# Agricultural-Robotics-Bonn/pagnerf

Hardware: AMD Instinct MI355X
Metric: rays/sec (train step) on BUP20-shape scene (higher is better)
Workload: dtype bf16

## Files before the change

### include/pagnerf_hip.h

```cpp
#ifndef PAGNERF_HIP_H
#define PAGNERF_HIP_H

#include <stdint.h>

#ifdef __cplusplus
extern "C" {
#endif

#define PAG_ABI_VERSION 14

enum { PAG_F32 = 0, PAG_F16 = 1, PAG_BF16 = 2 };
enum { PAG_OK = 0, PAG_ERR_ARG = -1, PAG_ERR_LAUNCH = -2, PAG_ERR_UNSUPPORTED = -3 };
enum { PAG_ACT_NONE = 0, PAG_ACT_SIGMOID = 1, PAG_ACT_SOFTMAX = 2 };
enum { PAG_MLP_MFMA_BF16 = 0, PAG_MLP_FP32 = 1 };
enum { PAG_BG_BLACK = 0, PAG_BG_WHITE = 1 };
enum { PAG_LAYOUT_STRIDED = 0, PAG_LAYOUT_XCD8 = 1 };
enum { PAG_ENC_HALF_COORDS = 1 };
#define PAG_MAX_LEVELS 32
#define PAG_MAX_FEATS 64

int pag_abi_version(void);
const char *pag_last_error_string(void);


// ... 91 lines not shown
    void *dz[3];
    void *dx1; int dx1_dtype;
    int mode;
    const float *g_ray; const float *g_scale; const int32_t *g_index;
    const float *softmax_stats; const float *b_last;
    int dx1_accumulate;
    const float *dx1_col0_add;
    const float *dx1_col0_gate;
    const float *g_ray_scale;
    const void *x1; int x1_dtype; const float *x2; int k2p; const int32_t *x2_index;
    float *wgrad_workspace; int64_t wgrad_workspace_bytes;
    float *dW[3]; float *db[3];
    const float *b[3];
    const struct pag_mlp_bwd_args *pair;
    float *dz0_slots;
} pag_mlp_bwd_args;
int pag_mlp_bwd(const pag_mlp_bwd_args *args, int64_t M, void *stream);
int64_t pag_mlp_dz0_slots_bytes(int64_t M, int64_t R);
int pag_mlp_dz0_slots_sum(const int64_t *pack_start, int64_t R, const float *slots, float *out, void *stream);
int pag_mlp_bwd_fused_supported(const pag_mlp_bwd_args *args);
#define PAG_MLP_FUSED_WIDE_MAX_M ((int64_t)1 << 24)
int64_t pag_mlp_bwd_fused_workspace_bytes(const pag_mlp_bwd_args *args, int64_t M);
int pag_mlp_bwd_pair_supported(const pag_mlp_bwd_args *args, const pag_mlp_bwd_args *pair);

int pag_affine_xcd8_fwd(const void *x, int64_t M, int x_levels, int x_feats, const float *W, const float *b, int n_out, int in_dim,
                        float *out, void *stream);
int pag_affine_xcd8_bwd_dx(const float *grad_out, int64_t M, int x_levels, int x_feats, const float *W, int n_out, int in_dim, void *dx,
                           void *stream);

int pag_head_composite_fwd(const int64_t *pack_start, const int32_t *ray_of_pack, int64_t P,
                           const void *hidden, const float *W_last, const float *b_last, int out_dim,
                           const float *softmax_stats, const float *weights, const float *alpha,
                           float *out, int64_t n_samples, void *stream);

int pag_mlp_wgrad_blocks(int64_t M);
int pag_mlp_wgrad(const void *dz, int dz_cols, int n_out, const void *a1, int a1_dtype,
                  int a1_layout, int k1, const float *a2, int k2p, const int32_t *a2_index, int n_in,
                  float *slabs, int n_blocks, int64_t M, void *stream);
// ... 290 lines not shown
```

### pagnerf_amd/_lib.py

```python
import ctypes
import os

import torch

from . import build as _build

F32, F16, BF16 = 0, 1, 2
I32, I64 = 3, 4
ACT_NONE, ACT_SIGMOID, ACT_SOFTMAX = 0, 1, 2
MLP_MFMA_BF16, MLP_FP32 = 0, 1
BG_BLACK, BG_WHITE = 0, 1
LAYOUT_STRIDED, LAYOUT_XCD8 = 0, 1
ENC_HALF_COORDS = 1
ABI_VERSION = 14
MLP_FUSED_WIDE_MAX_M = 1 << 24

_DT = {torch.float32: F32, torch.float16: F16, torch.bfloat16: BF16}

c_i64, c_i32, c_u32, c_f32, c_vp = ctypes.c_int64, ctypes.c_int, ctypes.c_uint32, ctypes.c_float, ctypes.c_void_p
c_fp = ctypes.POINTER(ctypes.c_float)
c_ip = ctypes.POINTER(ctypes.c_int)


class HeadCompositeArgs(ctypes.Structure):
# ... 31 lines not shown

MlpBwdArgs._fields_ = [("grad_out", c_vp), ("out", c_vp), ("out_dtype", c_i32), ("out_act", c_i32),
                ("k1", c_i32), ("in_dim", c_i32), ("n_layers", c_i32), ("out_dim", c_i32),
                ("x1_layout", c_i32), ("x1_levels", c_i32), ("x1_feats", c_i32),
                ("W", c_vp * 3),
                ("hidden_save", c_vp * 2),
                ("dz", c_vp * 3),
                ("dx1", c_vp), ("dx1_dtype", c_i32),
                ("mode", c_i32),
                ("g_ray", c_vp), ("g_scale", c_vp), ("g_index", c_vp),
                ("softmax_stats", c_vp), ("b_last", c_vp), ("dx1_accumulate", c_i32), ("dx1_col0_add", c_vp),
                ("dx1_col0_gate", c_vp), ("g_ray_scale", c_vp),
                ("x1", c_vp), ("x1_dtype", c_i32), ("x2", c_vp), ("k2p", c_i32), ("x2_index", c_vp),
                ("wgrad_workspace", c_vp), ("wgrad_workspace_bytes", c_i64),
                ("dW", c_vp * 3), ("db", c_vp * 3), ("b", c_vp * 3),
                ("pair", ctypes.POINTER(MlpBwdArgs)), ("dz0_slots", c_vp)]


class DeepMlpArgs(ctypes.Structure):
    _fields_ = [("coords", c_vp), ("ray_d", c_vp), ("hidden", c_i32), ("num_classes", c_i32), ("channels", c_i32), ("save", c_i32),
                ("W", c_vp * 14), ("b", c_vp * 14), ("density", c_vp), ("rgb", c_vp), ("semantics", c_vp),
                ("workspace", c_vp), ("workspace_bytes", c_i64),
                ("g_density", c_vp), ("g_rgb", c_vp), ("g_semantics", c_vp), ("dW", c_vp * 14), ("db", c_vp * 14),
                ("bwd_workspace", c_vp), ("bwd_workspace_bytes", c_i64)]


class VmArgs(ctypes.Structure):
    _fields_ = [("density_plane", c_vp * 3), ("density_line", c_vp * 3), ("app_plane", c_vp * 3), ("app_line", c_vp * 3), ("basis", c_vp),
                ("density_n_comp", c_i32), ("app_n_comp", c_i32), ("app_dim", c_i32), ("res", c_i32),
                ("xyz", c_vp), ("sigma", c_vp), ("app", c_vp), ("g_sigma", c_vp), ("g_app", c_vp),
                ("g_density_plane", c_vp * 3), ("g_density_line", c_vp * 3), ("g_app_plane", c_vp * 3), ("g_app_line", c_vp * 3), ("g_basis", c_vp),
# ... 17 lines not shown
    "pag_permuto_encode_bwd": (c_i32, [c_vp, c_i64, c_vp, c_i32, c_i64, c_i64, c_i32, c_i32, c_i32, c_u32, c_fp, c_fp, c_fp, c_vp, c_vp, c_i64, c_i32, c_vp]),
    "pag_permuto_encode_bwd_set": (c_i32, [c_vp, c_i64, c_vp, c_i32, c_i64, c_i64, c_i32, c_i32, c_i32, c_u32, c_fp, c_fp, c_fp, c_vp, c_vp, c_i64, c_i32, c_vp]),
    "pag_hash_encode_bwd_xyz": (c_i32, [c_vp, c_i64, c_vp, c_i32, c_vp, c_i32, c_i64, c_i64, c_i32, c_i32, c_i32, c_i32, c_fp, c_fp, c_vp, c_vp, c_i64, c_i32, c_vp]),
    "pag_permuto_encode_bwd_xyz": (c_i32, [c_vp, c_i64, c_vp, c_i32, c_vp, c_i32, c_i64, c_i64, c_i32, c_i32, c_i32, c_u32, c_fp, c_fp, c_fp, c_vp, c_vp, c_i64, c_i32, c_vp]),
    "pag_hash_encode_fwd_add": (c_i32, [c_vp, c_i64, c_vp, c_i32, c_i32, c_i32, c_i32, c_fp, c_fp, c_vp, c_vp, c_i32, c_vp]),
    "pag_permuto_encode_fwd_add": (c_i32, [c_vp, c_i64, c_vp, c_i32, c_i32, c_i32, c_u32, c_fp, c_fp, c_fp, c_vp, c_vp, c_i32, c_vp]),
    "pag_encode_bwd_workspace_bytes": (c_i64, [c_i64, c_i32, c_i32, c_i32, c_i64]),
    "pag_mlp_fwd": (c_i32, [ctypes.POINTER(MlpFwdArgs), c_i64, c_vp]),
    "pag_mlp_fwd_pair_supported": (c_i32, [ctypes.POINTER(MlpFwdArgs), ctypes.POINTER(MlpFwdArgs)]),
    "pag_mlp_fwd_composite_supported": (c_i32, [ctypes.POINTER(MlpFwdArgs), c_i64]),
    "pag_mlp_fwd_producer_supported": (c_i32, [ctypes.POINTER(MlpFwdArgs), ctypes.POINTER(MlpFwdArgs), c_i64]),
    "pag_mlp_bwd": (c_i32, [ctypes.POINTER(MlpBwdArgs), c_i64, c_vp]),
    "pag_mlp_bwd_fused_supported": (c_i32, [ctypes.POINTER(MlpBwdArgs)]),
    "pag_mlp_bwd_fused_workspace_bytes": (c_i64, [ctypes.POINTER(MlpBwdArgs), c_i64]),
    "pag_mlp_bwd_pair_supported": (c_i32, [ctypes.POINTER(MlpBwdArgs), ctypes.POINTER(MlpBwdArgs)]),
    "pag_head_composite_fwd": (c_i32, [c_vp, c_vp, c_i64, c_vp, c_vp, c_vp, c_i32, c_vp, c_vp, c_vp, c_vp, c_i64, c_vp]),
    "pag_mlp_wgrad_blocks": (c_i32, [c_i64]),
    "pag_mlp_wgrad_batch": (c_i32, [ctypes.POINTER(WgradLayer), c_i32, c_i64, c_vp]),
    "pag_mlp_wgrad_finish": (c_i32, [c_vp, c_i32, c_i32, c_i32, c_i32, c_i32, c_i32, c_vp, c_vp, c_vp]),
    "pag_mlp_wgrad": (c_i32, [c_vp, c_i32, c_i32, c_vp, c_i32, c_i32, c_i32, c_vp, c_i32, c_vp, c_i32, c_vp, c_i32, c_i64, c_vp]),
    "pag_raymarch_count": (c_i32, [c_vp, c_vp, c_i64, c_i32, c_vp, c_vp, c_f32, c_f32, c_vp, c_i32, c_vp, c_vp]),
    "pag_pack_offsets": (c_i32, [c_vp, c_i64, c_vp, c_vp, c_vp]),
    "pag_pad_packed": (c_i32, [c_vp, c_i64, c_i64, c_i32, c_vp, c_vp, c_vp, c_vp, c_vp, c_vp, c_vp, c_vp, c_vp, c_vp]),
    "pag_view_embed": (c_i32, [c_vp, c_i64, c_i32, c_i32, c_vp, c_vp]),
    "pag_raymarch_pack": (c_i32, [c_vp, c_vp, c_i64, c_i32, c_vp, c_vp, c_f32, c_f32, c_vp, c_i32, c_vp, c_vp, c_vp, c_vp, c_vp, c_vp, c_vp, c_vp, c_vp]),
    "pag_raymarch_voxel_count": (c_i32, [c_vp, c_vp, c_i64, c_i32, c_f32, c_f32, c_vp, c_vp, c_i32, c_f32, c_vp, c_vp]),
    "pag_raymarch_voxel_pack": (c_i32, [c_vp, c_vp, c_i64, c_i32, c_f32, c_f32, c_vp, c_vp, c_i32, c_f32, c_vp, c_vp, c_vp, c_vp, c_vp, c_vp, c_vp,
                                        c_vp, c_vp, c_vp]),
    "pag_raymarch_voxel_nugget_capacity": (c_i64, [c_i32]),
    "pag_raymarch_voxel_count_nuggets": (c_i32, [c_vp, c_vp, c_i64, c_i32, c_f32, c_f32, c_vp, c_vp, c_i32, c_f32, c_vp, c_vp, c_vp, c_vp]),
# ... 143 lines not shown
```

### pagnerf_amd/csrc/mlp.hip

```cpp
#include "mlp_common.h"

namespace {

constexpr int WIDE_BWD_WAVES = 8;
constexpr int RS = 72;
constexpr int HID = 64;

__device__ __forceinline__ int swap23(int a) { return (a & ~12) | ((a & 4) << 1) | ((a & 8) >> 1); }
struct FwdParams {
    const void *x1;
    const float *x2;
    const int32_t *x2_index;
    int k1, k2p, in_dim, in_pad, out_dim, act;
    const float *W[3];
    const float *b[3];
    void *out;
    void *hsave[2];
    int64_t M;
    int grp_L, grp_F;
    float *stats;
    float *col0_relu;
    const float *W2[2];
    const float *b2[2];
    void *out2;
// ... 2131 lines not shown
            constexpr bool S = bb >= 10;
            constexpr int k = S ? bb - 10 : bb - 4, ob = k >> 1, ib = k & 1;
            float *sl = (S ? ps.slabs[0] : pi.slabs[0]) + (int64_t)blockIdx.x * 64 * WG_SLAB_COLS;
#pragma unroll
            for (int q = 0; q < 16; ++q) {
                const float v = srcv(q);
                sl[(32 * ob + rho(q, h)) * WG_SLAB_COLS + 32 * ib + r] = v;
                if (ib == 1 && r == 31) sl[(32 * ob + rho(q, h)) * WG_SLAB_COLS + 64] = v;
            }
        } else {
#pragma unroll
            for (int q = 0; q < 16; ++q) {
                const float v = srcv(q);
                if (r < 2) pi.slabs[1][((int64_t)blockIdx.x * 64 + 32 * r + rho(q, h)) * WG_SLAB_COLS + 64] = v;
                if (r == 2) ps.slabs[1][((int64_t)blockIdx.x * 32 + rho(q, h)) * WG_SLAB_COLS + 64] = v;
            }
        }
    });
}

constexpr int WR_RS = 256;
constexpr int WB_RMAX = 4;
template <int OB>
__global__ __launch_bounds__((OB + 1) * 64) void mlp_bwd_wide_blocks(BwdParams p) {
    extern __shared__ __attribute__((aligned(16))) unsigned char smem[];
    constexpr int RSL = OB * 32 + 8;
    constexpr float LOG2E = 1.4426950408889634f;
    bf16_t *WLt = reinterpret_cast<bf16_t *>(smem);
    bf16_t *WLs = WLt + 64 * RSL;
    float *bLs = reinterpret_cast<float *>(WLs + OB * 32 * RS);
// ... 1382 lines not shown
        a->out_act == PAG_ACT_SIGMOID && a->out_dim <= 4 && a->dx1_col0_add && a->dx1_col0_gate && !a->dx1_accumulate)
        return 1;
    return -1;
}

extern "C" int pag_mlp_bwd_fused_supported(const pag_mlp_bwd_args *a) { return fused_kind(a) >= 0 ? 1 : 0; }

extern "C" int pag_mlp_bwd_pair_supported(const pag_mlp_bwd_args *a, const pag_mlp_bwd_args *b) {
    if (!a || !b || fused_kind(a) != 3 || fused_kind(b) != 2 || b->n_layers != 2) return 0;
    return (b->x1 == a->x1 && b->x1_layout == PAG_LAYOUT_XCD8 && b->x1_levels == a->x1_levels && b->x1_feats == a->x1_feats && b->in_dim == a->in_dim &&
            a->dx1 && b->dx1 == a->dx1 && b->dx1_accumulate && !a->dx1_accumulate)
               ? 1
               : 0;
}

extern "C" int64_t pag_mlp_bwd_fused_workspace_bytes(const pag_mlp_bwd_args *a, int64_t M) {
    const int kind = fused_kind(a);
    if (kind < 0 || M < 1) return 0;
    const int64_t grid = fused_grid(M);
    if (kind == 3)
        return (grid * 224 + grid * 128) * WG_SLAB_COLS * (int64_t)sizeof(float) + ((M + 31) / 32 + 1) * 32 * HID * 2;
    return grid * ((int64_t)(a->n_layers - 1) * 64 + 32) * WG_SLAB_COLS * (int64_t)sizeof(float);
}

extern "C" int pag_mlp_bwd(const pag_mlp_bwd_args *a, int64_t M, void *stream) {
    PAG_CHECK_ARG(a, "pag_mlp_bwd: args is NULL");
    PAG_CHECK_ARG(M >= 0, "pag_mlp_bwd: M < 0");
    PAG_CHECK_ARG(a->n_layers == 2 || a->n_layers == 3, "pag_mlp_bwd: n_layers %d not in {2,3}", a->n_layers);
    PAG_CHECK_ARG(a->k1 > 0 && a->k1 % 8 == 0 && a->k1 <= 64, "pag_mlp_bwd: k1 %d must be a multiple of 8 in (0,64]", a->k1);
    PAG_CHECK_ARG(a->in_dim > 0 && a->in_dim <= 64, "pag_mlp_bwd: in_dim %d out of range", a->in_dim);
    PAG_CHECK_ARG(a->out_dim >= 1 && a->out_dim <= 224, "pag_mlp_bwd: out_dim %d not in [1,224]", a->out_dim);
    PAG_CHECK_ARG(a->out_act >= PAG_ACT_NONE && a->out_act <= PAG_ACT_SOFTMAX, "pag_mlp_bwd: bad out_act %d", a->out_act);
    PAG_CHECK_ARG(a->out_act == PAG_ACT_NONE || a->out || (a->softmax_stats && a->b_last),
                  "pag_mlp_bwd: activated output (or softmax_stats + b_last) needed for sigmoid/softmax");
    PAG_CHECK_ARG(a->out_dtype == PAG_F32 || a->out_dtype == PAG_BF16, "pag_mlp_bwd: out dtype must be F32 or BF16");
    PAG_CHECK_ARG(a->dx1 == nullptr || a->dx1_dtype == PAG_F32 || a->dx1_dtype == PAG_BF16, "pag_mlp_bwd: dx1 dtype must be F32 or BF16");
    PAG_CHECK_ARG(a->mode == PAG_MLP_MFMA_BF16 || a->mode == PAG_MLP_FP32, "pag_mlp_bwd: bad mode %d", a->mode);
    if (M == 0) return PAG_OK;
    PAG_CHECK_ARG(a->grad_out || (a->g_ray && a->g_scale && a->g_index), "pag_mlp_bwd: NULL grad_out (and no rank-1 gradient)");
    PAG_CHECK_ARG(!a->g_ray || (a->mode == PAG_MLP_MFMA_BF16 && (a->out || a->softmax_stats)),
                  "pag_mlp_bwd: rank-1 gradients need MFMA mode and the saved output");
    const bool fuse = a->wgrad_workspace != nullptr;
    const int kind = fuse ? fused_kind(a) : -1;
    if (fuse) {
        PAG_CHECK_ARG(kind >= 0, "pag_mlp_bwd: this decoder shape has no fused weight-gradient kernel (pag_mlp_bwd_fused_supported)");
        PAG_CHECK_ARG(a->wgrad_workspace_bytes >= pag_mlp_bwd_fused_workspace_bytes(a, M), "pag_mlp_bwd: wgrad_workspace too small");
        for (int l = 0; l < a->n_layers; ++l) PAG_CHECK_ARG(a->dW[l] && a->db[l], "pag_mlp_bwd: NULL dW/db of layer %d", l);
        for (int l = 0; l + 1 < a->n_layers; ++l) PAG_CHECK_ARG(a->b[l], "pag_mlp_bwd: fused mode recomputes the hidden activations: NULL bias b[%d]", l);
    }
    for (int l = 0; l < a->n_layers; ++l) PAG_CHECK_ARG(a->W[l] && (fuse || a->dz[l]), "pag_mlp_bwd: NULL weight/dz of layer %d", l);
    for (int l = 0; l + 1 < a->n_layers; ++l)
        PAG_CHECK_ARG(a->hidden_save[l] || (a->wgrad_workspace && (a->out_dim <= 32 || l + 2 < a->n_layers)), "pag_mlp_bwd: NULL hidden_save[%d]", l);
    BwdParams p;
    p.g_ray = a->g_ray;
    p.g_scale = a->g_scale;
    p.g_ray_scale = a->g_ray_scale;
// ... 227 lines not shown
```

### pagnerf_amd/nef.py

```python
import copy
import inspect
import os

import numpy as np
import torch
import torch.nn as nn
import torch.nn.functional as F

from . import _lib as L
from . import ops
from .grids import HashGridHIP, PermutoGridHIP
from .triplanar import TriplanarGridHIP

_GRIDS = {"HashGridTorch": HashGridHIP, "HashGridTinyCudaNN": HashGridHIP, "HashGrid": HashGridHIP,
          "HashGridHIP": HashGridHIP, "PermutoGrid": PermutoGridHIP, "PermutoGridHIP": PermutoGridHIP,
          "TriplanarGrid": TriplanarGridHIP, "TriplanarGridHIP": TriplanarGridHIP}


class BasicDecoder(nn.Module):

    def __init__(self, input_dim, output_dim, num_layers=1, hidden_dim=64, bias=True):
        super().__init__()
        if hidden_dim != 64 or num_layers not in (1, 2):
            raise NotImplementedError("fused decoder supports hidden_dim=64 and 1-2 hidden layers (best.yaml); got %d x %d"
# ... 197 lines not shown
        out = {}
        if not compute_channels:
            return out
        if isinstance(compute_channels, str):
            compute_channels = {compute_channels}
        batch, num_samples, _ = coords.shape
        mode = self.mlp_mode
        pre = getattr(self, "_prefetched", None)
        self._prefetched = None
        if pre is not None and pre[0] is coords and pre[2] == torch.is_grad_enabled():
            feats = pre[1]
        else:
            feats = self._interp(self.grid, coords)
        self._feat_cache = (coords, feats if self._heads_read_live_features() else feats.detach())
        grp = self._grouped()
        hold = ops.decoder_hold(feats) if (ops.CD_FUSED and "rgb" in compute_channels and feats.is_cuda) else None
        try:
            density_feats = self.decoder_density(feats, mode=mode, out_dtype=self.feat_dtype, x1_grouped=grp)
            self._density_feats = density_feats.detach()
            if "rgb" in compute_channels:
                if num_samples != 1 and ridx is None:
                    ray_d = ray_d[:, None].repeat(1, num_samples, 1).reshape(-1, 3)
                pe, index = self._view_embedding(ray_d, ridx, ray_dirs)
                W, b = self.decoder_color.weights()
                rgb, sigma = ops.colour_and_density(density_feats, W, b, pe, index, self.decoder_color.input_dim, out_act=L.ACT_SIGMOID,
                                                    mode=mode, x2_packs=ray_packs if ridx is not None else None, producer=hold)
                density = sigma.reshape(batch, num_samples, 1)
                out["rgb"] = rgb.reshape(batch, num_samples, 3)
            else:
                density = torch.relu(density_feats[:, 0:1].float()).reshape(batch, num_samples, 1)
        finally:
            ops.flush_hold(hold)
        if "density" in compute_channels:
            out["density"] = density
        if "semantics" in compute_channels or "inst_embedding" in compute_channels:
            (sem_in, sem_grp), (inst_in, inst_grp) = self._head_inputs(feats, coords, compute_channels)
            if "semantics" in compute_channels:
                plain = not (self.sem_sigmoid or self.sem_normalize)
                act = L.ACT_SOFTMAX if (self.sem_softmax and plain) else L.ACT_NONE
                s = self.decoder_semantics(sem_in, out_act=act, mode=mode, x1_grouped=sem_grp, out_dtype=self.feat_dtype)
                if not plain:
                    s = torch.sigmoid(s) if self.sem_sigmoid else s
                    s = F.normalize(s, dim=-1) if self.sem_normalize else s
                    s = F.softmax(s, dim=-1) if self.sem_softmax else s
                out["semantics"] = s
            if "inst_embedding" in compute_channels:
                out["inst_embedding"] = self._inst_head(inst_in, inst_grp, mode)
# ... 152 lines not shown
```

### pagnerf_amd/ops.py

```python
import ctypes
import os
import threading
import time

import torch

from . import _lib as L


_PROFILE = None


_PROFILE_ONLY = None


def profile_start(only=None):
    global _PROFILE, _PROFILE_ONLY
    _PROFILE = {}
    _PROFILE_ONLY = set(only) if only is not None else None


def profile_stop():
    global _PROFILE
    prof, _PROFILE = _PROFILE, None
# ... 479 lines not shown
        ctx.out_dtype = out_dtype
        extra = (stats, bc[-1]) if stats is not None else ()
        ctx.save_for_backward(x1, x2, x2_index, out, *hidden, *Wc, *extra)
        ctx.n_hidden = len(hidden)
        ctx.bc = bc
        if stats_only:
            ctx.fwd_state = (hidden[-1], Wc[-1], bc[-1], stats)
        return out

    @staticmethod
    def backward(ctx, g):
        return _FusedMLP._backward_impl(ctx, g, None)

    @staticmethod
    def _backward_impl(ctx, g, rank1, dx1_into=None, col0_add=None, col0_gate=None, wgrad_queue=None, dx1_out=None, hold=None,
                       pair_hold=None):
        lib = L.load()
        in_dim, out_act, mode, n_layers, k1, grouped = ctx.cfg
        saved = ctx.saved_tensors
        x1, x2, x2_index, out = saved[:4]
        hidden = list(saved[4:4 + ctx.n_hidden])
        Wc = list(saved[4 + ctx.n_hidden:4 + ctx.n_hidden + n_layers])
        stats, b_last = (saved[-2], saved[-1]) if getattr(ctx, "has_stats", False) else (None, None)
        M = x1.shape[1] if grouped is not None else x1.shape[0]
        out_dim = Wc[-1].shape[0]
        dev = x1.device
        zdt = torch.bfloat16 if mode == L.MLP_MFMA_BF16 else torch.float32
        out_dtype = ctx.out_dtype
        need_dx = ctx.needs_input_grad[0]
        need_dx2 = ctx.needs_input_grad[1] and x2 is not None
        dx1 = (dx1_into if dx1_into is not None else (dx1_out if dx1_out is not None else torch.empty(x1.shape, device=dev, dtype=x1.dtype))) \
# ... 59 lines not shown
                gW.append(torch.empty(Wc[l].shape[0], in_dim if l == 0 else 64, device=dev))
                gb.append(torch.empty(Wc[l].shape[0], device=dev))
                a.dW[l], a.db[l] = L.ptr(gW[l]), L.ptr(gb[l])
        else:
            dz = [torch.empty(M, 64, device=dev, dtype=zdt) for _ in range(n_layers - 1)] + [torch.empty(M, out_dim, device=dev, dtype=zdt)]
            for i in range(n_layers):
                a.dz[i] = L.ptr(dz[i])
        if M and hold is not None:
            hold["args"], hold["M"], hold["fused"] = a, M, fused
            hold["keep"] = [v for v in locals().values() if isinstance(v, (torch.Tensor, list, tuple))]
        elif M:
            if pair_hold is not None and fused and pair_hold.get("fused") \
                    and lib.pag_mlp_bwd_pair_supported(ctypes.byref(a), ctypes.byref(pair_hold["args"])) == 1:
                a.pair = ctypes.pointer(pair_hold["args"])
                pair_hold["taken"] = True
            _call("pag_mlp_bwd", ctypes.byref(a), M, L.stream())
        if col0_add is not None and need_dx and not fuse_col0:
            dx1[:, 0] += col0_add.to(dx1.dtype)
        if fused:
            pass
        elif mode == L.MLP_MFMA_BF16 and M:
            specs = []
            for l in range(n_layers):
                n_out = Wc[l].shape[0]
                sp = dict(dz=dz[l], n_out=n_out, a2=None, k2p=0, a2_index=None, levels=0, feats=0)
                if l == 0 and grouped is not None:
                    sp.update(a1=x1, a1_dtype=L.BF16, a1_layout=L.LAYOUT_XCD8, k1=64, n_in=64, levels=grouped[0], feats=grouped[1])
                elif l == 0:
                    sp.update(a1=x1, a1_dtype=L.dtype_code(x1), a1_layout=L.LAYOUT_STRIDED, k1=k1, n_in=in_dim,
                              a2=x2, k2p=(x2.shape[1] if x2 is not None else 0), a2_index=x2_index)
# ... 119 lines not shown
        return rgb, torch.relu(pre)

    @staticmethod
    def backward(ctx, g_rgb, g_sigma):
        saved_out = ctx.saved_tensors[3]
        if g_rgb is None:
            g_rgb = torch.zeros_like(saved_out)
        if g_sigma is None:
            return _FusedMLP._backward_impl(ctx, g_rgb, None)
        if ctx.pre is None:
            return _FusedMLP._backward_impl(ctx, g_rgb, None, col0_add=g_sigma.float().contiguous(), col0_gate=ctx.col0_relu)
        add = (g_sigma.float() * (ctx.pre > 0)).contiguous()
        return _FusedMLP._backward_impl(ctx, g_rgb, None, col0_add=add)


def colour_and_density(x1, weights, biases, x2, x2_index, in_dim, out_act=L.ACT_SIGMOID, mode=L.MLP_MFMA_BF16,
                       out_dtype=torch.float32, x2_packs=None, producer=None):
    global _NEXT_PRODUCER
    _NEXT_PRODUCER = producer
    try:
        rgb, sigma = _apply_decoder(_ColourDensity, x1, x2, x2_index, int(in_dim), out_act, mode, out_dtype, None, *weights, *biases)
    finally:
        _NEXT_PRODUCER = None
    if x2_packs is not None and x2 is not None and x2.requires_grad and rgb.grad_fn is not None:
        rgb.grad_fn.x2_packs = x2_packs
    return rgb, sigma


def fused_mlp(x1, weights, biases, x2=None, x2_index=None, in_dim=None, out_act=L.ACT_NONE, mode=L.MLP_MFMA_BF16,
              out_dtype=torch.float32, x1_grouped=None, x2_packs=None):
# ... 567 lines not shown
                    s3[lo:hi, 0] = (feats[lo:hi].float() * g[rl[lo:hi]]).sum(1)
                ones = torch.zeros(alpha.shape[0], 3, device=dev)
                ones[:, 0] = 1.0
                d_rgb = torch.empty(M, 3, device=dev)
                _call("pag_composite_bwd", L.ptr(pack_start), L.ptr(ray_of_pack), P, L.ptr(sigma), L.ptr(deltas), None, L.ptr(s3),
                      L.BG_BLACK, L.ptr(w), L.ptr(alpha), L.ptr(ones), None, None, L.ptr(d_sigma), L.ptr(d_rgb), 0, L.stream())
        return d_sigma, None, (d_feats if ctx.needs_input_grad[2] else None), None, None, None, None


def composite_features(sigma, deltas, feats, ridx, pack_start, ray_of_pack, N):
    return _apply(_CompositeFeatsWeights, sigma, deltas, feats, ridx, pack_start, ray_of_pack, N)


HEAD_REBUILD = True
CD_FUSED = os.environ.get("PAG_CD_FUSED", "1") != "0"
_NEXT_HOLD = None
_NEXT_PRODUCER = None


def decoder_hold(x1):
    global _NEXT_HOLD
    _NEXT_HOLD = {"x1_ptr": x1.data_ptr()}
    return _NEXT_HOLD


def flush_hold(hold):
    global _NEXT_HOLD, _NEXT_PRODUCER
    if _NEXT_HOLD is hold:
        _NEXT_HOLD = None
    if hold is not None and _NEXT_PRODUCER is hold:
# ... 313 lines not shown
```

Baseline: 1.216 million.

## Fuse colour and density decoder backward into a single kernel launch

Adds a combined backward kernel that recomputes both decoders' hidden activations and runs the colour decoder's backward straight into the density decoder's backward per tile. The colour decoder's dx1 stays in registers and feeds the density decoder, and the weight gradients of both are accumulated in one pass. A new autograd Function wires forward and backward together when the feature, grad and dtype conditions hold. This removes a launch and the round trip of the intermediate density-feature gradient through global memory, at the cost of much higher LDS and register pressure in one large kernel.

```diff
diff --git a/include/pagnerf_hip.h b/include/pagnerf_hip.h
--- a/include/pagnerf_hip.h
+++ b/include/pagnerf_hip.h
@@ -129,6 +129,7 @@
     const float *b[3];
     const struct pag_mlp_bwd_args *pair;
     float *dz0_slots;
+    const struct pag_mlp_bwd_args *x1_producer;
 } pag_mlp_bwd_args;
 int pag_mlp_bwd(const pag_mlp_bwd_args *args, int64_t M, void *stream);
 int64_t pag_mlp_dz0_slots_bytes(int64_t M, int64_t R);
@@ -137,6 +138,7 @@
 #define PAG_MLP_FUSED_WIDE_MAX_M ((int64_t)1 << 24)
 int64_t pag_mlp_bwd_fused_workspace_bytes(const pag_mlp_bwd_args *args, int64_t M);
 int pag_mlp_bwd_pair_supported(const pag_mlp_bwd_args *args, const pag_mlp_bwd_args *pair);
+int pag_mlp_bwd_producer_supported(const pag_mlp_bwd_args *args, const pag_mlp_bwd_args *producer, int64_t M);
 
 int pag_affine_xcd8_fwd(const void *x, int64_t M, int x_levels, int x_feats, const float *W, const float *b, int n_out, int in_dim,
                         float *out, void *stream);
diff --git a/pagnerf_amd/_lib.py b/pagnerf_amd/_lib.py
--- a/pagnerf_amd/_lib.py
+++ b/pagnerf_amd/_lib.py
@@ -69,7 +69,7 @@
                 ("x1", c_vp), ("x1_dtype", c_i32), ("x2", c_vp), ("k2p", c_i32), ("x2_index", c_vp),
                 ("wgrad_workspace", c_vp), ("wgrad_workspace_bytes", c_i64),
                 ("dW", c_vp * 3), ("db", c_vp * 3), ("b", c_vp * 3),
-                ("pair", ctypes.POINTER(MlpBwdArgs)), ("dz0_slots", c_vp)]
+                ("pair", ctypes.POINTER(MlpBwdArgs)), ("dz0_slots", c_vp), ("x1_producer", ctypes.POINTER(MlpBwdArgs))]
 
 
 class DeepMlpArgs(ctypes.Structure):
@@ -117,6 +117,7 @@
     "pag_mlp_bwd_fused_supported": (c_i32, [ctypes.POINTER(MlpBwdArgs)]),
     "pag_mlp_bwd_fused_workspace_bytes": (c_i64, [ctypes.POINTER(MlpBwdArgs), c_i64]),
     "pag_mlp_bwd_pair_supported": (c_i32, [ctypes.POINTER(MlpBwdArgs), ctypes.POINTER(MlpBwdArgs)]),
+    "pag_mlp_bwd_producer_supported": (c_i32, [ctypes.POINTER(MlpBwdArgs), ctypes.POINTER(MlpBwdArgs), c_i64]),
     "pag_head_composite_fwd": (c_i32, [c_vp, c_vp, c_i64, c_vp, c_vp, c_vp, c_i32, c_vp, c_vp, c_vp, c_vp, c_i64, c_vp]),
     "pag_mlp_wgrad_blocks": (c_i32, [c_i64]),
     "pag_mlp_wgrad_batch": (c_i32, [ctypes.POINTER(WgradLayer), c_i32, c_i64, c_vp]),
diff --git a/pagnerf_amd/csrc/mlp.hip b/pagnerf_amd/csrc/mlp.hip
--- a/pagnerf_amd/csrc/mlp.hip
+++ b/pagnerf_amd/csrc/mlp.hip
@@ -2169,6 +2169,333 @@
                 const float v = srcv(q);
                 if (r < 2) pi.slabs[1][((int64_t)blockIdx.x * 64 + 32 * r + rho(q, h)) * WG_SLAB_COLS + 64] = v;
                 if (r == 2) ps.slabs[1][((int64_t)blockIdx.x * 32 + rho(q, h)) * WG_SLAB_COLS + 64] = v;
+            }
+        }
+    });
+}
+
+struct CdParams {
+    BwdParams c, d;
+};
+__global__ __launch_bounds__(256, 1) void mlp_bwd_colour_density(CdParams pp) {
+    const BwdParams &pc = pp.c, &pd = pp.d;
+    extern __shared__ __attribute__((aligned(16))) unsigned char smem[];
+    constexpr int RSL = 40;
+    bf16_t *WLtC = reinterpret_cast<bf16_t *>(smem);
+    bf16_t *W1tC = WLtC + 64 * RSL;
+    bf16_t *W0tC = W1tC + 64 * RS;
+    bf16_t *W0sC = W0tC + 64 * RS;
+    bf16_t *W1sC = W0sC + 64 * RS;
+    bf16_t *WLtD = W1sC + 64 * RS;
+    bf16_t *W0tD = WLtD + 64 * RSL;
+    bf16_t *W0sD = W0tD + 64 * RS;
+    float *b0C = reinterpret_cast<float *>(W0sD + 64 * RS);
+    float *b1C = b0C + 64, *b0D = b1C + 64;
+    stage_weight_t(WLtC, RSL, 64, 32, pc.W[2], pc.out_dim, HID);
+    stage_weight_both(W0sC, RS, false, W0tC, RS, 64, 64, pc.W[0], HID, pc.in_dim);
+    stage_weight_both(W1sC, RS, true, W1tC, RS, 64, 64, pc.W[1], HID, HID);
+    stage_weight_t(WLtD, RSL, 64, 32, pd.W[1], pd.out_dim, HID);
+    stage_weight_both(W0sD, RS, false, W0tD, RS, 64, 64, pd.W[0], HID, pd.in_dim, pd.grp_L, pd.grp_F);
+    for (int e = threadIdx.x; e < 64; e += blockDim.x) {
+        b0C[e] = pc.b[0][e];
+        b1C[e] = pc.b[1][e];
+        b0D[e] = pd.b[0][e];
+    }
+    bf16_t *Tx = reinterpret_cast<bf16_t *>(b0D + 64) + (threadIdx.x >> 6) * (5 * TW_ELEMS);
+    bf16_t *Th0 = Tx + TW_ELEMS, *Th1 = Th0 + TW_ELEMS, *Tz = Th1 + TW_ELEMS, *TxD = Tz + TW_ELEMS;
+    bf16_t *ThD = Th1;
+    __syncthreads();
+
+    const int lane = threadIdx.x & 63, wave = threadIdx.x >> 6;
+    const int r = lane & 31, h = lane >> 5;
+    const int64_t M = pc.M, ntiles = (M + 31) / 32, nfull = M / 32;
+    const int64_t tile_step = (int64_t)gridDim.x * 4;
+    const bf16_t *x1c = reinterpret_cast<const bf16_t *>(pc.x1), *x1d = reinterpret_cast<const bf16_t *>(pd.x1);
+    const int32_t *ridx = pc.x2_index;
+
+    bf16x8 xnc[3], xnd[4];
+    float gs[4], gy[4], c0a = 0.0f;
+    int ray1 = 0, ray2 = 0;
+    auto row_of = [&](int64_t tile) __attribute__((always_inline)) { return min(min(tile, ntiles - 1) * 32 + r, M - 1); };
+    auto prefetch_c = [&](int64_t tile_raw, int ray) __attribute__((always_inline)) {
+        const unsigned m = (unsigned)row_of(tile_raw);
+        xnc[0] = load8(x1c + (m * 16u + 8u * h));
+        xnc[1] = load8(pc.x2 + ((unsigned)ray * 32u + 8u * h));
+        xnc[2] = load8(pc.x2 + ((unsigned)ray * 32u + 16u + 8u * h));
+        const float *gop = reinterpret_cast<const float *>(pc.grad_out) + m * (unsigned)pc.out_dim;
+        const float *yop = reinterpret_cast<const float *>(pc.out) + m * (unsigned)pc.out_dim;
+#pragma unroll
+        for (int j = 0; j < 4; ++j) {
+            const int c = j < pc.out_dim ? j : 0;
+            gs[j] = gop[c];
+            gy[j] = yop[c];
+        }
+        c0a = pc.dx_col0[m];
+    };
+    auto prefetch_d = [&](int64_t tile_raw) __attribute__((always_inline)) {
+        const unsigned off = ((unsigned)h * (unsigned)M + (unsigned)row_of(tile_raw)) * 8u;
+#pragma unroll
+        for (int s = 0; s < 4; ++s) xnd[s] = load8(x1d + (int64_t)(2 * s) * M * 8 + off);
+    };
+
+    f32x16 awLC[1][2], awMC[2][2], aw0C[2][2], awLD[1][2], aw0D[2][2], dbacc;
+#pragma unroll
+    for (int q = 0; q < 16; ++q) {
+        dbacc[q] = 0.0f;
+#pragma unroll
+        for (int i = 0; i < 2; ++i) {
+            awLC[0][i][q] = awLD[0][i][q] = 0.0f;
+#pragma unroll
+            for (int j = 0; j < 2; ++j) awMC[i][j][q] = aw0C[i][j][q] = aw0D[i][j][q] = 0.0f;
+        }
+    }
+    auto ones_col = [&](int j) __attribute__((always_inline)) {
+        bf16x8 o;
+#pragma unroll
+        for (int e = 0; e < 8; ++e) o[e] = (bf16_t)(r == j ? 1.0f : 0.0f);
+        return o;
+    };
+    auto wgrad_tile = [&](const bf16_t *Tin, auto &aw, int dbcol) __attribute__((always_inline)) {
+        constexpr int NOB = (int)(sizeof(aw) / sizeof(aw[0]));
+#pragma unroll
+        for (int ks = 0; ks < 2; ++ks) {
+            bf16x8 bfr[2], afr[NOB];
+#pragma unroll
+            for (int ib = 0; ib < 2; ++ib) bfr[ib] = tw_frag(Tin, ib, ks, lane);
+#pragma unroll
+            for (int ob = 0; ob < NOB; ++ob) afr[ob] = tw_frag(Tz, ob, ks, lane);
+#pragma unroll
+            for (int ob = 0; ob < NOB; ++ob) {
+#pragma unroll
+                for (int ib = 0; ib < 2; ++ib) aw[ob][ib] = __builtin_amdgcn_mfma_f32_32x32x16_bf16(afr[ob], bfr[ib], aw[ob][ib], 0, 0, 0);
+                if (dbcol >= 0) dbacc = __builtin_amdgcn_mfma_f32_32x32x16_bf16(afr[ob], ones_col(dbcol + ob), dbacc, 0, 0, 0);
+            }
+        }
+    };
+    bf16x4 pend[2][4];
+#pragma unroll
+    for (int mb = 0; mb < 2; ++mb)
+#pragma unroll
+        for (int g = 0; g < 4; ++g) pend[mb][g] = bf16x4{(bf16_t)0.0f, (bf16_t)0.0f, (bf16_t)0.0f, (bf16_t)0.0f};
+    unsigned pend_m = (unsigned)min((int64_t)blockIdx.x * 4 * 32 + (int64_t)wave * 32 + r, M - 1);
+    auto flush = [&](bool pred) __attribute__((always_inline)) {
+#pragma unroll
+        for (int mb = 0; mb < 2; ++mb)
+#pragma unroll
+            for (int g = 0; g < 4; ++g) {
+                bf16_t *dst = reinterpret_cast<bf16_t *>(pd.dx1) + (int64_t)(4 * mb + g) * M * 8 + (pend_m * 8u + 4u * h);
+                if (pred) *reinterpret_cast<bf16x4 *>(dst) = pend[mb][g];
+            }
+    };
+    auto body = [&](int64_t tile, auto full_tag) __attribute__((always_inline)) {
+        constexpr bool FULL = decltype(full_tag)::value;
+        const int64_t m = tile * 32 + r;
+        const bool live = FULL || m < M;
+        f32x16 acc[2];
+        bf16x8 hb[4];
+        wave_lds_sync();
+        const float col0 = (h == 0 && (float)xnc[0][0] > 0.0f) ? c0a : 0.0f;
+        {
+            bf16x8 xb[4];
+#pragma unroll
+            for (int s = 0; s < 3; ++s) xb[s] = xnc[s];
+            xb[3] = zero8();
+            if (h == 1) xb[3][7] = (bf16_t)1.0f;
+            tw_put_frags(Tx, xb, r, h);
+            {
+                bf16x8 xd[4];
+#pragma unroll
+                for (int s = 0; s < 4; ++s) xd[s] = xnd[s];
+                if (h == 1) xd[3][7] = (bf16_t)1.0f;
+                tw_put_frags(TxD, xd, r, h);
+            }
+            f32x16 ha[2];
+            bf16x8 hf[4];
+            hidden_layer_pinned<4>(W0sC, b0C, xb, r, h, ha);
+#pragma unroll
+            for (int mb = 0; mb < 2; ++mb) {
+#pragma unroll
+                for (int q = 0; q < 16; ++q) ha[mb][q] = fmaxf(ha[mb][q], 0.0f);
+                tw_put_block(Th0, mb, r, h, ha[mb]);
+                pack_block(ha[mb], hf[2 * mb], hf[2 * mb + 1]);
+            }
+            hidden_layer_pinned<4>(W1sC, b1C, hf, r, h, ha);
+#pragma unroll
+            for (int mb = 0; mb < 2; ++mb) {
+#pragma unroll
+                for (int q = 0; q < 16; ++q) ha[mb][q] = fmaxf(ha[mb][q], 0.0f);
+                tw_put_block(Th1, mb, r, h, ha[mb]);
+            }
+        }
+        {
+            f32x16 z;
+#pragma unroll
+            for (int q = 0; q < 16; ++q) z[q] = 0.0f;
+#pragma unroll
+            for (int j = 0; j < 4; ++j) {
+                const float y = gy[j];
+                z[j] = (h == 0 && j < pc.out_dim && live) ? gs[j] * y * (1.0f - y) : 0.0f;
+            }
+            flush(true);
+            prefetch_c(tile + tile_step, ray1);
+            ray1 = ray2;
+            ray2 = ridx[row_of(tile + 3 * tile_step)];
+            bf16x8 zb[2];
+            pack_block(z, zb[0], zb[1]);
+            tw_put_block(Tz, 0, r, h, z);
+            wave_lds_sync();
+            wgrad_tile(Th1, awLC, 0);
+            wave_lds_sync();
+            wt_chain_pinned<2, 2>(WLtC, RSL, zb, r, h, acc);
+            relu_mask_pack_put(Th1, Tz, r, h, live, acc, hb);
+            wave_lds_sync();
+        }
+        {
+            bf16x8 hb2[4];
+            wgrad_tile(Th0, awMC, 1);
+            wave_lds_sync();
+            wt_chain_pinned<2, 4>(W1tC, RS, hb, r, h, acc);
+            relu_mask_pack_put(Th0, Tz, r, h, live, acc, hb2);
+            wave_lds_sync();
+            wgrad_tile(Tx, aw0C, -1);
+            wt_chain_pinned<1, 4>(W0tC, RS, hb2, r, h, acc);
+        }
+        acc[0][0] += col0;
+        bf16x4 g16[2];
+#pragma unroll
+        for (int g = 0; g < 2; ++g) g16[g] = bf16x4{(bf16_t)acc[0][4 * g], (bf16_t)acc[0][4 * g + 1], (bf16_t)acc[0][4 * g + 2], (bf16_t)acc[0][4 * g + 3]};
+        wave_lds_sync();
+        prefetch_d(tile + tile_step);
+        {
+            bf16x8 xb[4];
+#pragma unroll
+            for (int s = 0; s < 4; ++s) {
+                const bf16x4 lo = *reinterpret_cast<const bf16x4 *>(TxD + tw_off(r, 4 * s + 2 * h)), hi = *reinterpret_cast<const bf16x4 *>(TxD + tw_off(r, 4 * s + 2 * h + 1));
+                xb[s] = bf16x8{lo[0], lo[1], lo[2], lo[3], hi[0], hi[1], hi[2], hi[3]};
+            }
+            f32x16 ha[2];
+            hidden_layer_pinned<4>(W0sD, b0D, xb, r, h, ha);
+#pragma unroll
+            for (int mb = 0; mb < 2; ++mb) {
+#pragma unroll
+                for (int q = 0; q < 16; ++q) ha[mb][q] = fmaxf(ha[mb][q], 0.0f);
+                tw_put_block(ThD, mb, r, h, ha[mb]);
+            }
+        }
+        {
+            f32x16 z;
+#pragma unroll
+            for (int g = 0; g < 4; ++g)
+#pragma unroll
+                for (int j = 0; j < 4; ++j) z[4 * g + j] = (g < 2 && live) ? (float)g16[g & 1][j] : 0.0f;
+            bf16x8 zb[2];
+            pack_block(z, zb[0], zb[1]);
+            tw_put_block(Tz, 0, r, h, z);
+            wave_lds_sync();
+            wgrad_tile(ThD, awLD, 3);
+            wave_lds_sync();
+            wt_chain_pinned<2, 2>(WLtD, RSL, zb, r, h, acc);
+            relu_mask_pack_put(ThD, Tz, r, h, live, acc, hb);
+            wave_lds_sync();
+        }
+        wgrad_tile(TxD, aw0D, -1);
+        wt_chain_pinned<2, 4>(W0tD, RS, hb, r, h, acc);
+#pragma unroll
+        for (int mb = 0; mb < 2; ++mb)
+#pragma unroll
+            for (int g = 0; g < 4; ++g)
+                pend[mb][g] = bf16x4{(bf16_t)acc[mb][4 * g], (bf16_t)acc[mb][4 * g + 1], (bf16_t)acc[mb][4 * g + 2], (bf16_t)acc[mb][4 * g + 3]};
+        pend_m = (unsigned)min(m, M - 1);
+    };
+
+    int64_t tile = (int64_t)blockIdx.x * 4 + wave;
+    const int ray0 = ridx[row_of(tile)];
+    ray1 = ridx[row_of(tile + tile_step)];
+    ray2 = ridx[row_of(tile + 2 * tile_step)];
+    prefetch_c(tile, ray0);
+    prefetch_d(tile);
+    const bool any_tile = tile < ntiles;
+    bool last_ragged = false;
+    for (; tile < nfull; tile += tile_step) body(tile, std::true_type{});
+    if (tile < ntiles) {
+        body(tile, std::false_type{});
+        last_ragged = true;
+    }
+    if (any_tile) flush(!last_ragged || (nfull * 32 + r) < M);
+
+    constexpr int NBLK = 2 + 4 + 4 + 2 + 4 + 1;
+    auto blk = [&](auto bi) -> const f32x16 & {
+        constexpr int bb = decltype(bi)::value;
+        if constexpr (bb < 2) return awLC[0][bb];
+        else if constexpr (bb < 6) return awMC[(bb - 2) >> 1][(bb - 2) & 1];
+        else if constexpr (bb < 10) return aw0C[(bb - 6) >> 1][(bb - 6) & 1];
+        else if constexpr (bb < 12) return awLD[0][bb - 10];
+        else if constexpr (bb < 16) return aw0D[(bb - 12) >> 1][(bb - 12) & 1];
+        else return dbacc;
+    };
+    __syncthreads();
+    float *red = reinterpret_cast<float *>(smem);
+    if (wave == 0) {
+        static_for<NBLK>([&](auto bi) {
+            constexpr int bb = decltype(bi)::value;
+            const f32x16 &a = blk(bi);
+            f32x4 *dst = reinterpret_cast<f32x4 *>(red) + (bb * 4) * 64 + lane;
+#pragma unroll
+            for (int q4 = 0; q4 < 4; ++q4) dst[q4 * 64] = f32x4{a[4 * q4], a[4 * q4 + 1], a[4 * q4 + 2], a[4 * q4 + 3]};
+        });
+    }
+    __syncthreads();
+#pragma unroll 1
+    for (int w = 1; w < 4; ++w) {
+        if (wave == w) {
+            static_for<NBLK>([&](auto bi) {
+                constexpr int bb = decltype(bi)::value;
+                const f32x16 &a = blk(bi);
+                f32x4 *dst = reinterpret_cast<f32x4 *>(red) + (bb * 4) * 64 + lane;
+                f32x4 t[4];
+#pragma unroll
+                for (int q4 = 0; q4 < 4; ++q4) t[q4] = dst[q4 * 64];
+#pragma unroll
+                for (int q4 = 0; q4 < 4; ++q4) dst[q4 * 64] = t[q4] + f32x4{a[4 * q4], a[4 * q4 + 1], a[4 * q4 + 2], a[4 * q4 + 3]};
+            });
+        }
+        __syncthreads();
+    }
+    static_for<NBLK>([&](auto bi) {
+        constexpr int bb = decltype(bi)::value;
+        if ((bb & 3) != wave) return;
+        f32x4 sv[4];
+#pragma unroll
+        for (int q4 = 0; q4 < 4; ++q4) sv[q4] = (reinterpret_cast<const f32x4 *>(red) + (bb * 4 + q4) * 64 + lane)[0];
+        auto srcv = [&](int q) __attribute__((always_inline)) { return sv[q >> 2][q & 3]; };
+        if constexpr (bb < 2 || (bb >= 10 && bb < 12)) {
+            constexpr bool D = bb >= 10;
+            constexpr int ib = D ? bb - 10 : bb;
+            float *sl = (D ? pd.slabs[1] : pc.slabs[2]) + (int64_t)blockIdx.x * 32 * WG_SLAB_COLS;
+#pragma unroll
+            for (int q = 0; q < 16; ++q) sl[rho(q, h) * WG_SLAB_COLS + 32 * ib + r] = srcv(q);
+        } else if constexpr (bb < 6) {
+            constexpr int ob = (bb - 2) >> 1, ib = (bb - 2) & 1;
+            float *sl = pc.slabs[1] + (int64_t)blockIdx.x * 64 * WG_SLAB_COLS;
+#pragma unroll
+            for (int q = 0; q < 16; ++q) sl[(32 * ob + rho(q, h)) * WG_SLAB_COLS + 32 * ib + r] = srcv(q);
+        } else if constexpr (bb < 16) {
+            constexpr bool D = bb >= 12;
+            constexpr int k = D ? bb - 12 : bb - 6, ob = k >> 1, ib = k & 1;
+            float *sl = (D ? pd.slabs[0] : pc.slabs[0]) + (int64_t)blockIdx.x * 64 * WG_SLAB_COLS;
+#pragma unroll
+            for (int q = 0; q < 16; ++q) {
+                const float v = srcv(q);
+                sl[(32 * ob + rho(q, h)) * WG_SLAB_COLS + 32 * ib + r] = v;
+                if (ib == 1 && r == 31) sl[(32 * ob + rho(q, h)) * WG_SLAB_COLS + 64] = v;
+            }
+        } else {
+#pragma unroll
+            for (int q = 0; q < 16; ++q) {
+                const float v = srcv(q);
+                if (r == 0) pc.slabs[2][((int64_t)blockIdx.x * 32 + rho(q, h)) * WG_SLAB_COLS + 64] = v;
+                if (r == 1 || r == 2) pc.slabs[1][((int64_t)blockIdx.x * 64 + 32 * (r - 1) + rho(q, h)) * WG_SLAB_COLS + 64] = v;
+                if (r == 3) pd.slabs[1][((int64_t)blockIdx.x * 32 + rho(q, h)) * WG_SLAB_COLS + 64] = v;
             }
         }
     });
@@ -3581,6 +3908,64 @@
                : 0;
 }
 
+extern "C" int pag_mlp_bwd_producer_supported(const pag_mlp_bwd_args *a, const pag_mlp_bwd_args *d, int64_t M) {
+    if (!a || !d || M < 1 || M > PAG_MLP_FUSED_WIDE_MAX_M || fused_kind(a) != 1 || fused_kind(d) != 0) return 0;
+    if (a->n_layers != 3 || d->n_layers != 2 || d->out_dim != 16 || a->pair || d->pair || d->x1_producer) return 0;
+    if (a->dz[0] || a->dz0_slots) return 0;
+    if (d->grad_out != a->dx1) return 0;
+    for (int l = 0; l < 3; ++l)
+        if (!a->W[l] || !a->dW[l] || !a->db[l] || (l < 2 && (!a->b[l] || !d->W[l] || !d->dW[l] || !d->db[l]))) return 0;
+    return (d->b[0] && a->wgrad_workspace && d->wgrad_workspace && a->wgrad_workspace_bytes >= pag_mlp_bwd_fused_workspace_bytes(a, M) &&
+            d->wgrad_workspace_bytes >= pag_mlp_bwd_fused_workspace_bytes(d, M))
+               ? 1
+               : 0;
+}
+
+static int launch_bwd_colour_density(const pag_mlp_bwd_args *a, const pag_mlp_bwd_args *d, int64_t M, hipStream_t st) {
+    const unsigned grid = fused_grid(M);
+    CdParams pp{};
+    const pag_mlp_bwd_args *blocks[2] = {a, d};
+    BwdParams *ps[2] = {&pp.c, &pp.d};
+    FinishBatch fb{};
+    int n_fin = 0;
+    for (int k = 0; k < 2; ++k) {
+        const pag_mlp_bwd_args *s = blocks[k];
+        BwdParams &p = *ps[k];
+        p.grad_out = s->grad_out;
+        p.out = s->out;
+        p.k1 = s->k1;
+        p.in_dim = s->in_dim;
+        p.in_pad = 64;
+        p.out_dim = s->out_dim;
+        p.act = s->out_act;
+        p.M = M;
+        p.grp_L = s->x1_layout == PAG_LAYOUT_XCD8 ? s->x1_levels : 0;
+        p.grp_F = s->x1_feats;
+        p.x1 = s->x1;
+        p.x2 = s->x2;
+        p.x2_index = s->x2_index;
+        p.k2p = s->x2 ? s->k2p : 0;
+        p.dx1 = s->dx1;
+        p.dx_col0 = s->dx1_col0_add;
+        float *ws = s->wgrad_workspace;
+        for (int l = 0; l < s->n_layers; ++l) {
+            p.W[l] = s->W[l];
+            p.b[l] = s->b[l];
+            p.slabs[l] = ws;
+            ws += (int64_t)grid * (l + 1 < s->n_layers ? 64 : 32) * WG_SLAB_COLS;
+            const int n_out = l + 1 < s->n_layers ? HID : s->out_dim;
+            fb.p[n_fin++] = FinishParams{p.slabs[l], (int)grid, n_out, (n_out + 31) / 32 * 32, l == 0 ? s->in_dim : HID, l == 0 ? p.grp_L : 0, p.grp_F, s->dW[l], s->db[l]};
+        }
+    }
+    const size_t lds = (size_t)(2 * 64 * 40 + 6 * 64 * RS) * sizeof(bf16_t) + 192 * sizeof(float) + (size_t)4 * 5 * TW_ELEMS * sizeof(bf16_t);
+    raise_lds_limit<mlp_bwd_colour_density>();
+    hipLaunchKernelGGL(mlp_bwd_colour_density, dim3(grid), dim3(256), lds, st, pp);
+    PAG_CHECK_LAUNCH("pag_mlp_bwd (fused, colour + density)");
+    launch_wgrad_finish(fb, HID, n_fin, st);
+    PAG_CHECK_LAUNCH("pag_mlp_bwd (fused, finish)");
+    return PAG_OK;
+}
+
 extern "C" int64_t pag_mlp_bwd_fused_workspace_bytes(const pag_mlp_bwd_args *a, int64_t M) {
     const int kind = fused_kind(a);
     if (kind < 0 || M < 1) return 0;
@@ -3607,6 +3992,11 @@
     PAG_CHECK_ARG(a->grad_out || (a->g_ray && a->g_scale && a->g_index), "pag_mlp_bwd: NULL grad_out (and no rank-1 gradient)");
     PAG_CHECK_ARG(!a->g_ray || (a->mode == PAG_MLP_MFMA_BF16 && (a->out || a->softmax_stats)),
                   "pag_mlp_bwd: rank-1 gradients need MFMA mode and the saved output");
+    if (a->x1_producer) {
+        PAG_CHECK_ARG(pag_mlp_bwd_producer_supported(a, a->x1_producer, M) == 1,
+                      "pag_mlp_bwd: x1_producer is not supported for these arguments (pag_mlp_bwd_producer_supported)");
+        return launch_bwd_colour_density(a, a->x1_producer, M, (hipStream_t)stream);
+    }
     const bool fuse = a->wgrad_workspace != nullptr;
     const int kind = fuse ? fused_kind(a) : -1;
     if (fuse) {
diff --git a/pagnerf_amd/nef.py b/pagnerf_amd/nef.py
--- a/pagnerf_amd/nef.py
+++ b/pagnerf_amd/nef.py
@@ -235,14 +235,31 @@
             feats = self._interp(self.grid, coords)
         self._feat_cache = (coords, feats if self._heads_read_live_features() else feats.detach())
         grp = self._grouped()
+        pe_index = None
+        if (ops.CD_FUSED and ops.CD_BWD_FUSED and "rgb" in compute_channels and feats.is_cuda and grp is not None and mode == L.MLP_MFMA_BF16
+                and torch.is_grad_enabled() and feats.requires_grad and feats.dtype == torch.bfloat16):
+            if num_samples != 1 and ridx is None:
+                ray_d = ray_d[:, None].repeat(1, num_samples, 1).reshape(-1, 3)
+            pe_index = self._view_embedding(ray_d, ridx, ray_dirs)
+            if not pe_index[0].requires_grad:
+                Wd, bd = self.decoder_density.weights()
+                W, b = self.decoder_color.weights()
+                rgb, sigma, self._density_feats = ops.density_and_colour(feats, grp, (Wd, bd, self.decoder_density.input_dim),
+                                                                         (W, b, self.decoder_color.input_dim), pe_index[0], pe_index[1], mode=mode,
+                                                                         feat_dtype=self.feat_dtype)
+                out["rgb"] = rgb.reshape(batch, num_samples, 3)
+                return self._rgb_semantics_heads(out, sigma.reshape(batch, num_samples, 1), feats, coords, compute_channels, mode)
         hold = ops.decoder_hold(feats) if (ops.CD_FUSED and "rgb" in compute_channels and feats.is_cuda) else None
         try:
             density_feats = self.decoder_density(feats, mode=mode, out_dtype=self.feat_dtype, x1_grouped=grp)
             self._density_feats = density_feats.detach()
             if "rgb" in compute_channels:
-                if num_samples != 1 and ridx is None:
-                    ray_d = ray_d[:, None].repeat(1, num_samples, 1).reshape(-1, 3)
-                pe, index = self._view_embedding(ray_d, ridx, ray_dirs)
+                if pe_index is not None:
+                    pe, index = pe_index
+                else:
+                    if num_samples != 1 and ridx is None:
+                        ray_d = ray_d[:, None].repeat(1, num_samples, 1).reshape(-1, 3)
+                    pe, index = self._view_embedding(ray_d, ridx, ray_dirs)
                 W, b = self.decoder_color.weights()
                 rgb, sigma = ops.colour_and_density(density_feats, W, b, pe, index, self.decoder_color.input_dim, out_act=L.ACT_SIGMOID,
                                                     mode=mode, x2_packs=ray_packs if ridx is not None else None, producer=hold)
@@ -252,6 +269,9 @@
                 density = torch.relu(density_feats[:, 0:1].float()).reshape(batch, num_samples, 1)
         finally:
             ops.flush_hold(hold)
+        return self._rgb_semantics_heads(out, density, feats, coords, compute_channels, mode)
+
+    def _rgb_semantics_heads(self, out, density, feats, coords, compute_channels, mode):
         if "density" in compute_channels:
             out["density"] = density
         if "semantics" in compute_channels or "inst_embedding" in compute_channels:
diff --git a/pagnerf_amd/ops.py b/pagnerf_amd/ops.py
--- a/pagnerf_amd/ops.py
+++ b/pagnerf_amd/ops.py
@@ -517,7 +517,7 @@
 
     @staticmethod
     def _backward_impl(ctx, g, rank1, dx1_into=None, col0_add=None, col0_gate=None, wgrad_queue=None, dx1_out=None, hold=None,
-                       pair_hold=None):
+                       pair_hold=None, producer_hold=None):
         lib = L.load()
         in_dim, out_act, mode, n_layers, k1, grouped = ctx.cfg
         saved = ctx.saved_tensors
@@ -607,6 +607,10 @@
                     and lib.pag_mlp_bwd_pair_supported(ctypes.byref(a), ctypes.byref(pair_hold["args"])) == 1:
                 a.pair = ctypes.pointer(pair_hold["args"])
                 pair_hold["taken"] = True
+            if producer_hold is not None and fused and producer_hold.get("fused") and CD_BWD_FUSED \
+                    and lib.pag_mlp_bwd_producer_supported(ctypes.byref(a), ctypes.byref(producer_hold["args"]), M) == 1:
+                a.x1_producer = ctypes.pointer(producer_hold["args"])
+                producer_hold["taken"] = True
             _call("pag_mlp_bwd", ctypes.byref(a), M, L.stream())
         if col0_add is not None and need_dx and not fuse_col0:
             dx1[:, 0] += col0_add.to(dx1.dtype)
@@ -756,6 +760,55 @@
         return _FusedMLP._backward_impl(ctx, g_rgb, None, col0_add=add)
 
 
+class _DensityColour(torch.autograd.Function):
+
+    @staticmethod
+    def forward(ctx, feats, x2, x2_index, grouped, mode, feat_dtype, in_dims, n_d, *wb):
+        global _NEXT_HOLD, _NEXT_PRODUCER
+        any_grad = any(ctx.needs_input_grad)
+        sub_d, sub_c = _SubCtx(ctx.needs_input_grad[0], any_grad), _SubCtx(True, any_grad)
+        hold = {"x1_ptr": feats.data_ptr()}
+        try:
+            _NEXT_HOLD = hold
+            dens = _FusedMLP.forward(sub_d, feats, None, None, in_dims[0], L.ACT_NONE, mode, feat_dtype, grouped, *wb[:n_d])
+            _NEXT_PRODUCER = hold
+            rgb, sigma = _ColourDensity.forward(sub_c, dens, x2, x2_index, in_dims[1], L.ACT_SIGMOID, mode, torch.float32, None, *wb[n_d:])
+        finally:
+            _NEXT_PRODUCER = None
+            flush_hold(hold)
+        ctx.one_launch = all(c.n_hidden > 0 and all(h is None for h in c.saved_tensors[4:4 + c.n_hidden]) for c in (sub_d, sub_c)) \
+            and sub_c.pre is None and sub_c.col0_relu is not None
+        ctx.subs = (sub_d, sub_c)
+        ctx.mark_non_differentiable(dens)
+        return rgb, sigma, dens
+
+    @staticmethod
+    def backward(ctx, g_rgb, g_sigma, _g_dens):
+        sub_d, sub_c = ctx.subs
+        if g_rgb is None:
+            g_rgb = torch.zeros_like(sub_c.saved_tensors[3])
+        x1 = sub_c.saved_tensors[0]
+        if CD_BWD_FUSED and ctx.one_launch and g_sigma is not None and x1.shape[0] and sub_d.needs_input_grad[0]:
+            dx1 = torch.empty(x1.shape, device=x1.device, dtype=x1.dtype)
+            hold = {}
+            gd = _FusedMLP._backward_impl(sub_d, dx1, None, hold=hold)
+            if not hold.get("fused"):
+                raise RuntimeError("pagnerf_amd: the density decoder's backward has no fused kernel although its forward skipped the hidden activations")
+            gc = _FusedMLP._backward_impl(sub_c, g_rgb, None, col0_add=g_sigma.float().contiguous(), col0_gate=sub_c.col0_relu, dx1_out=dx1,
+                                          producer_hold=hold)
+            if not hold.get("taken"):
+                _call("pag_mlp_bwd", ctypes.byref(hold["args"]), hold["M"], L.stream())
+        else:
+            gc = _ColourDensity.backward(sub_c, g_rgb, g_sigma)
+            gd = _FusedMLP._backward_impl(sub_d, gc[0], None)
+        return (gd[0], gc[1], None, None, None, None, None, None, *gd[8:], *gc[8:])
+
+
+def density_and_colour(feats, grouped, density, colour, x2, x2_index, mode=L.MLP_MFMA_BF16, feat_dtype=torch.bfloat16):
+    (wd, bd, i_d), (wc, bc, i_c) = density, colour
+    return _apply_decoder(_DensityColour, feats, x2, x2_index, grouped, mode, feat_dtype, (int(i_d), int(i_c)), len(wd) + len(bd), *wd, *bd, *wc, *bc)
+
+
 def colour_and_density(x1, weights, biases, x2, x2_index, in_dim, out_act=L.ACT_SIGMOID, mode=L.MLP_MFMA_BF16,
                        out_dtype=torch.float32, x2_packs=None, producer=None):
     global _NEXT_PRODUCER
@@ -1353,6 +1406,7 @@
 
 HEAD_REBUILD = True
 CD_FUSED = os.environ.get("PAG_CD_FUSED", "1") != "0"
+CD_BWD_FUSED = os.environ.get("PAG_CD_BWD_FUSED", "1") != "0"
 _NEXT_HOLD = None
 _NEXT_PRODUCER = None
 
```

After: 1.215 million, median of 2. About the same (-0.0%).
